# rapidsai/cugraph

Measured on NVIDIA H100. Metric: MTEPS (million traversed edges/sec) PageRank RMAT-24 ef-16, 100 iterations, higher is better.
Workload: dtype f32

## Files before the change

cugraph_b200/csrc/capi_basic.cu:

```cuda
#include "graph.cuh"

#include <cstdlib>
#include <map>
#include <mutex>
#include <unordered_map>
#include <unordered_set>

namespace b200 {
namespace {
std::mutex g_stream_mutex;
std::unordered_map<cudaStream_t, int>& live_streams()
{
  static auto* s = new std::unordered_map<cudaStream_t, int>();
  return *s;
}
struct block_cache_t {
  std::multimap<size_t, void*> blocks;
  size_t total{0};
};
std::unordered_map<cudaStream_t, block_cache_t>& block_caches()
{
  static auto* c = new std::unordered_map<cudaStream_t, block_cache_t>();
  return *c;
}
// ... 37 lines not shown
    cudaDeviceSynchronize();
    e = cudaMallocAsync(&p, bytes, s);
  }
  CUDA_TRY(e);
  *capacity = bytes;
  return p;
}

void block_free(void* p, size_t capacity, cudaStream_t s)
{
  std::lock_guard<std::mutex> lk(g_stream_mutex);
  if (live_streams().count(s) == 0) {
    cudaFree(p);
    return;
  }
  block_cache_t& c = block_caches()[s];
  if (c.total + capacity > kBlockCacheCap) flush_cache_locked(s, c, true);
  if (capacity > kBlockCacheCap) {
    cudaFreeAsync(p, s);
    return;
  }
  c.blocks.emplace(capacity, p);
  c.total += capacity;
}

bool stream_is_live(cudaStream_t s)
{
  std::lock_guard<std::mutex> lk(g_stream_mutex);
  return live_streams().count(s) != 0;
}
void register_stream(cudaStream_t s)
{
  std::lock_guard<std::mutex> lk(g_stream_mutex);
  ++live_streams()[s];
}
void unregister_stream(cudaStream_t s)
{
  std::lock_guard<std::mutex> lk(g_stream_mutex);
  auto live = live_streams().find(s);
  if (live != live_streams().end() && --live->second > 0) return;
  auto it = block_caches().find(s);
  if (it != block_caches().end()) {
    flush_cache_locked(s, it->second, true);
    block_caches().erase(it);
  }
  live_streams().erase(s);
}

namespace {
struct handle_deleter {
  void operator()(handle_impl* h) const
  {
    if (h->pinned) cudaFreeHost(h->pinned);
    if (h->stream && !h->borrowed_stream) cudaStreamDestroy(h->stream);
    delete h;
  }
};

cugraph_resource_handle_t* create_handle(const char* entry, cudaStream_t stream, bool borrowed)
{
  try {
    std::unique_ptr<handle_impl, handle_deleter> h(new handle_impl{});
    h->tune            = tuning_t::from_env();
    h->stream          = stream;
    h->borrowed_stream = borrowed;
    CUDA_TRY(cudaGetDevice(&h->device));
    if (!borrowed) CUDA_TRY(cudaStreamCreateWithFlags(&h->stream, cudaStreamNonBlocking));
    cudaDeviceProp prop{};
    CUDA_TRY(cudaGetDeviceProperties(&prop, h->device));
    h->sm_count = prop.multiProcessorCount;
    h->l2_bytes = static_cast<size_t>(prop.l2CacheSize);
    CUDA_TRY(cudaMallocHost(&h->pinned, 4096));
    cudaMemPool_t pool;
    CUDA_TRY(cudaDeviceGetDefaultMemPool(&pool, h->device));
    uint64_t threshold = UINT64_MAX;
    CUDA_TRY(cudaMemPoolSetAttribute(pool, cudaMemPoolAttrReleaseThreshold, &threshold));
    register_stream(h->stream);
    return reinterpret_cast<cugraph_resource_handle_t*>(h.release());
  } catch (std::exception const& e) {
    std::fprintf(stderr, "%s: %s\n", entry, e.what());
    return nullptr;
  }
}
}
}

using namespace b200;

extern "C" {

const char* cugraph_error_message(const cugraph_error_t* error)
{
  if (error == nullptr) return nullptr;
  return reinterpret_cast<error_impl const*>(error)->message.c_str();
}

void cugraph_error_free(cugraph_error_t* error)
{
  if (error != nullptr) delete reinterpret_cast<error_impl*>(error);
}

cugraph_resource_handle_t* cugraph_create_resource_handle(void* raft_handle)
{
  if (raft_handle != nullptr) {
    std::fprintf(stderr, "cugraph_create_resource_handle: multi-GPU goes through cugraph_b200.mg (torch.distributed) + the "
                         "cugraph_b200_block_* entry points\n");
    return nullptr;
  }
  return create_handle("cugraph_create_resource_handle", nullptr, false);
}

int cugraph_resource_handle_get_comm_size(const cugraph_resource_handle_t*) { return 1; }

int cugraph_resource_handle_get_rank(const cugraph_resource_handle_t*) { return 0; }

void cugraph_free_resource_handle(cugraph_resource_handle_t* handle)
{
  if (!handle) return;
  auto* h = reinterpret_cast<handle_impl*>(handle);
  cudaStreamSynchronize(h->stream);
// ... 248 lines not shown
```

cugraph_b200/csrc/common.cuh:

```cuda
#pragma once

#include <cugraph_c/b200_ext.h>
#include <cugraph_c/graph_functions.h>
#include <cugraph_c/labeling_algorithms.h>
#include <cuda_runtime.h>

#include <algorithm>
#include <cstdint>
#include <cstdio>
#include <cstdlib>
#include <cstring>
#include <stdexcept>
#include <string>
#include <utility>

namespace b200 {

struct error_impl {
  std::string message;
};

struct capi_exception : public std::runtime_error {
  cugraph_error_code_t code;
  capi_exception(cugraph_error_code_t c, std::string const& m) : std::runtime_error(m), code(c) {}
// ... 9 lines not shown
    cudaError_t e__ = (call);                                                                    \
    if (e__ != cudaSuccess) {                                                                    \
      cudaGetLastError();                                                                        \
      throw ::b200::capi_exception(                                                              \
        e__ == cudaErrorMemoryAllocation ? CUGRAPH_ALLOC_ERROR : CUGRAPH_UNKNOWN_ERROR,          \
        std::string("CUDA error ") + cudaGetErrorName(e__) + " at " + __FILE__ + ":" +           \
          std::to_string(__LINE__) + ": " + cudaGetErrorString(e__));                            \
    }                                                                                            \
  } while (0)

template <typename F>
cugraph_error_code_t guarded(cugraph_error_t** error, F&& f)
{
  if (error) *error = nullptr;
  try {
    f();
    return CUGRAPH_SUCCESS;
  } catch (capi_exception const& e) {
    if (error) *error = reinterpret_cast<cugraph_error_t*>(new error_impl{e.what()});
    return e.code;
  } catch (std::bad_alloc const&) {
    if (error) *error = reinterpret_cast<cugraph_error_t*>(new error_impl{"host allocation failed"});
    return CUGRAPH_ALLOC_ERROR;
  } catch (std::exception const& e) {
    if (error) *error = reinterpret_cast<cugraph_error_t*>(new error_impl{e.what()});
    return CUGRAPH_UNKNOWN_ERROR;
  }
}

inline size_t dtype_size(cugraph_data_type_id_t t)
{
  switch (t) {
    case INT8:
    case UINT8:
    case BOOL: return 1;
    case INT16:
    case UINT16: return 2;
    case INT32:
    case UINT32:
    case FLOAT32: return 4;
    case INT64:
    case UINT64:
    case FLOAT64:
    case SIZE_T: return 8;
    default: return 0;
  }
}

struct tuning_t {
  long long sweep_min_edges{1ll << 22};
  bool sweep_bank_order{true};
  int sweep_bands{0};
  int sweep_tail_degree{0};
  double bfs_alpha{40.0}, bfs_beta{24.0};
  bool sssp_adaptive{true};
  double sssp_delta_scale{1.0};
  double sssp_start_div{64.0};
  bool sssp_small_rounds{true};
  int sssp_split_rounds{1};
  unsigned long long sssp_split_min_edges{1ull << 20};
  unsigned long long advance_split_edges{1ull << 31};
  long long offs64_min_edges{1ll << 31};
  bool bfs_trace{false}, sssp_trace{false}, build_trace{false}, scc_trace{false};
  static tuning_t from_env()
  {
    tuning_t t;
    auto get = [](const char* k) { return std::getenv(k); };
    if (auto e = get("CUGRAPH_B200_SWEEP_MIN_EDGES")) t.sweep_min_edges = std::atoll(e);
    if (auto e = get("CUGRAPH_B200_SWEEP_BANK_ORDER")) t.sweep_bank_order = std::atoi(e) != 0;
    if (auto e = get("CUGRAPH_B200_SWEEP_BANDS")) t.sweep_bands = std::max(0, std::atoi(e));
    if (auto e = get("CUGRAPH_B200_SWEEP_TAIL_DEGREE")) t.sweep_tail_degree = std::max(0, std::atoi(e));
    if (auto e = get("CUGRAPH_B200_BFS_ALPHA")) t.bfs_alpha = std::atof(e);
    if (auto e = get("CUGRAPH_B200_BFS_BETA")) t.bfs_beta = std::atof(e);
    if (auto e = get("CUGRAPH_B200_SSSP_ADAPTIVE")) t.sssp_adaptive = std::atoi(e) != 0;
    if (auto e = get("CUGRAPH_B200_SSSP_DELTA_SCALE")) t.sssp_delta_scale = std::atof(e);
    if (auto e = get("CUGRAPH_B200_SSSP_START_DIV")) t.sssp_start_div = std::max(1.0, std::atof(e));
    if (auto e = get("CUGRAPH_B200_SSSP_SMALL_ROUNDS")) t.sssp_small_rounds = std::atoi(e) != 0;
    if (auto e = get("CUGRAPH_B200_SSSP_SPLIT_ROUNDS")) t.sssp_split_rounds = std::max(1, std::atoi(e));
    if (auto e = get("CUGRAPH_B200_SSSP_SPLIT_MIN_EDGES")) t.sssp_split_min_edges = std::strtoull(e, nullptr, 10);
    if (auto e = get("CUGRAPH_B200_ADVANCE_SPLIT_EDGES")) t.advance_split_edges = std::min<unsigned long long>(std::max<unsigned long long>(std::strtoull(e, nullptr, 10), 2ull), 1ull << 31);
    if (auto e = get("CUGRAPH_B200_OFFS64_MIN_EDGES")) t.offs64_min_edges = std::min(std::max(std::atoll(e), 0ll), 1ll << 31);
    t.bfs_trace   = get("CUGRAPH_B200_BFS_TRACE") != nullptr;
    t.sssp_trace  = get("CUGRAPH_B200_SSSP_TRACE") != nullptr;
    t.build_trace = get("CUGRAPH_B200_BUILD_TRACE") != nullptr;
    t.scc_trace   = get("CUGRAPH_B200_SCC_TRACE") != nullptr;
    return t;
  }
};

struct handle_impl {
  tuning_t tune{};
  int device{0};
  cudaStream_t stream{nullptr};
  bool borrowed_stream{false};
  int sm_count{132};
  size_t l2_bytes{0};
  mutable size_t launches{0};
  void* pinned{nullptr};
};

inline handle_impl const& H(const cugraph_resource_handle_t* h)
{
  B200_EXPECTS(h != nullptr, CUGRAPH_INVALID_HANDLE, "resource handle is NULL");
  return *reinterpret_cast<handle_impl const*>(h);
}

inline bool bfs_bottom_up(handle_impl const& h, bool bottom_up, long long n_f, long long prev_n_f, unsigned long long m_f,
                          unsigned long long m_u, long long n_unvisited)
{
  if (!bottom_up && (double)m_f * h.tune.bfs_alpha > (double)m_u && n_f >= prev_n_f) return true;
  if (bottom_up && (double)n_f * h.tune.bfs_beta < (double)n_unvisited && n_f < prev_n_f) return false;
  return bottom_up;
}

bool stream_is_live(cudaStream_t s);
void register_stream(cudaStream_t s);
void unregister_stream(cudaStream_t s);

void* block_alloc(size_t bytes, cudaStream_t s, size_t* capacity);
void block_free(void* p, size_t capacity, cudaStream_t s);

class dbuf {
 public:
  dbuf() = default;
  dbuf(size_t bytes, cudaStream_t s) : bytes_(bytes), stream_(s)
  {
    if (bytes_ > 0) p_ = block_alloc(bytes_, s, &cap_);
  }
  dbuf(dbuf const&)            = delete;
  dbuf& operator=(dbuf const&) = delete;
  dbuf(dbuf&& o) noexcept { swap(o); }
  dbuf& operator=(dbuf&& o) noexcept
  {
    if (this != &o) {
      release();
      swap(o);
    }
    return *this;
  }
  ~dbuf() { release(); }
  void release()
  {
    if (p_) block_free(p_, cap_, stream_);
    p_     = nullptr;
    bytes_ = cap_ = 0;
  }
  void* data() const { return p_; }
// ... 40 lines not shown
};

struct host_array_view_impl {
  void* data{nullptr};
  size_t size{0};
  cugraph_data_type_id_t type{INT32};
  size_t nbytes() const { return size * dtype_size(type); }
};

struct host_array_impl {
  void* data{nullptr};
  size_t size{0};
  cugraph_data_type_id_t type{INT32};
};

inline device_array_view_impl const* V(const cugraph_type_erased_device_array_view_t* v)
{
  return reinterpret_cast<device_array_view_impl const*>(v);
}

inline cugraph_type_erased_device_array_t* wrap_array(dbuf&& b, size_t n, cugraph_data_type_id_t t)
{
  auto* a = new device_array_impl{std::move(b), n, t};
  return reinterpret_cast<cugraph_type_erased_device_array_t*>(a);
}

struct centrality_result_impl {
  device_array_impl* vertices{nullptr};
  device_array_impl* values{nullptr};
  size_t iterations{0};
  bool converged{false};
};

struct paths_result_impl {
  device_array_impl* vertices{nullptr};
  device_array_impl* distances{nullptr};
  device_array_impl* predecessors{nullptr};
};

struct labeling_result_impl {
  device_array_impl* vertices{nullptr};
  device_array_impl* labels{nullptr};
};

constexpr int kBlock = 256;

inline int grid_for(int64_t n, int per_thread = 1, int max_grid = 1 << 20)
{
  const int64_t b = (n + (int64_t)kBlock * per_thread - 1) / ((int64_t)kBlock * per_thread);
  return (int)std::min<int64_t>(std::max<int64_t>(b, 1), std::min(max_grid, 1 << 20));
}

#ifndef B200_HOST_EMU
#define B200_LAUNCH(h, kernel, grid, block, smem, ...)                           \
  do {                                                                           \
    if ((grid) > 0) {                                                            \
      kernel<<<(grid), (block), (smem), (h).stream>>>(__VA_ARGS__);              \
      (h).launches++;                                                            \
    }                                                                            \
  } while (0)
__device__ __forceinline__ bool is_commit_lane() { return (threadIdx.x & 31) == 0; }
#else
#define B200_LAUNCH(h, kernel, grid, block, smem, ...)                           \
  do {                                                                           \
    if ((grid) > 0) {                                                            \
      emu_launch((grid), (block), (size_t)(smem), [&] { kernel(__VA_ARGS__); }); \
      (h).launches++;                                                            \
    }                                                                            \
  } while (0)
inline bool is_commit_lane() { return true; }
#endif

__device__ __forceinline__ double warp_sum(double v)
{
#pragma unroll
  for (int o = 16; o > 0; o >>= 1) v += __shfl_xor_sync(0xffffffffu, v, o);
  return v;
}

inline void check_last(const char* what)
{
  cudaError_t e = cudaGetLastError();
  if (e != cudaSuccess)
    throw capi_exception(CUGRAPH_UNKNOWN_ERROR,
                         std::string("kernel launch failed (") + what + "): " + cudaGetErrorString(e));
}

inline void sync(handle_impl const& h) { CUDA_TRY(cudaStreamSynchronize(h.stream)); }

template <typename T>
T read_back(handle_impl const& h, T const* d)
{
  T v{};
  CUDA_TRY(cudaMemcpyAsync(&v, d, sizeof(T), cudaMemcpyDeviceToHost, h.stream));
  sync(h);
  return v;
}

namespace {

template <typename T>
__global__ void k_fill(T* __restrict__ a, int64_t n, T v)
{
  for (int64_t i = blockIdx.x * (int64_t)blockDim.x + threadIdx.x; i < n; i += (int64_t)gridDim.x * blockDim.x) a[i] = v;
}

template <typename T>
__global__ void k_iota(T* __restrict__ a, int64_t n)
{
  for (int64_t i = blockIdx.x * (int64_t)blockDim.x + threadIdx.x; i < n; i += (int64_t)gridDim.x * blockDim.x) a[i] = (T)i;
}

template <typename T>
__global__ void k_count_negative(T const* __restrict__ a, int64_t n, int* __restrict__ out)
{
  for (int64_t i = blockIdx.x * (int64_t)blockDim.x + threadIdx.x; i < n; i += (int64_t)gridDim.x * blockDim.x)
    if (a[i] < (T)0) atomicAdd(out, 1);
}

__device__ __forceinline__ double block_sum(double v, double* smem)
{
  v = warp_sum(v);
  if ((threadIdx.x & 31) == 0) smem[threadIdx.x >> 5] = v;
  __syncthreads();
// ... 45 lines not shown
```

cugraph_b200/csrc/sweep.cuh:

```cuda
#pragma once
#include "spmv.cuh"
#include "sweep_layout.cuh"

namespace b200 {

constexpr int kSweepThreads = 512;
constexpr int kSweepWarps   = kSweepThreads / 32;
constexpr int kSweepDynSmem = kHotSliceBytes;
constexpr int kTmaPiece     = 16 * 1024;
constexpr int kStealMin     = 12;

#ifndef B200_HOST_EMU
__device__ __forceinline__ uint32_t smem_u32(const void* p) { return (uint32_t)__cvta_generic_to_shared(p); }

__device__ __forceinline__ void mbar_init(uint64_t* bar, unsigned count)
{
  asm volatile("mbarrier.init.shared::cta.b64 [%0], %1;" ::"r"(smem_u32(bar)), "r"(count));
  asm volatile("fence.mbarrier_init.release.cluster;" ::: "memory");
}
__device__ __forceinline__ void mbar_expect_tx(uint64_t* bar, unsigned bytes)
{
  asm volatile("mbarrier.arrive.expect_tx.shared::cta.b64 _, [%0], %1;" ::"r"(smem_u32(bar)), "r"(bytes) : "memory");
}
__device__ __forceinline__ void mbar_wait(uint64_t* bar, unsigned parity)
// ... 559 lines not shown
    else if (r < n_cov) acc[r] = 0.0;
    const T v0 = (T)(q[k].x * alpha + init), v1 = (T)(q[k].y * alpha + init);
    bool paired = false;
    if constexpr (sizeof(T) == 4) {
      if (!row_vertex && r + 1 < n_rows) {
        if (y) *reinterpret_cast<float2*>(y + r) = make_float2(v0, v1);
        if (epi.x_next) epi_row_pair(epi, r, v0, v1, make_float2((float)ow[k][0], (float)ow[k][1]), sums);
        paired = true;
      }
    }
    if (!paired) {
#pragma unroll
      for (int j = 0; j < 2; ++j) {
        if (r + j < n_rows) {
          const int v = row_vertex ? row_vertex[r + j] : r + j;
          store_row(y, epi, v, j ? v1 : v0, epi_in_t<T>{ow[k][j], epi.y_old ? epi.y_old[v] : (T)0}, sums);
        }
      }
    }
  }
  epi_flush(epi, sums);
}

constexpr int kTailThreads = 512;
constexpr int kTailBatch   = 8;

#ifndef B200_HOST_EMU
__device__ __forceinline__ float ld_keep(float const* p, unsigned long long pol)
{
  float v;
  asm("ld.global.nc.L2::cache_hint.f32 %0, [%1], %2;" : "=f"(v) : "l"(p), "l"(pol));
  return v;
}
__device__ __forceinline__ double ld_keep(double const* p, unsigned long long pol)
{
  double v;
  asm("ld.global.nc.L2::cache_hint.f64 %0, [%1], %2;" : "=d"(v) : "l"(p), "l"(pol));
  return v;
}
#else
inline float ld_keep(float const* p, unsigned long long) { return *p; }
inline double ld_keep(double const* p, unsigned long long) { return *p; }
#endif

template <typename T>
struct tail_args_t {
  tail_run_t const* __restrict__ runs;
  int32_t const* __restrict__ ids;
  T const* __restrict__ w;
  T const* __restrict__ x;
  T* __restrict__ y;
  int32_t const* __restrict__ row_vertex;
  int* __restrict__ cursor;
  pr_state_t const* __restrict__ st;
  int n_runs, empty_hi, W;
  double alpha;
  row_epi_t<T> epi;
};

struct tail_unit_t {
  int d, n_tiles, row0, row_end;
  long long base;
};

__device__ __forceinline__ tail_unit_t tail_unit(tail_run_t const* runs, int n_runs, int u)
{
  tail_unit_t t{0, 0, 0, 0, 0};
  if (u >= runs[n_runs].first_unit) return t;
  int r = 0;
  while (u >= runs[r + 1].first_unit) ++r;
  const tail_run_t R = runs[r];
  const int per      = tail_unit_tiles(R.degree);
  const int tile     = (u - R.first_unit) * per;
  t.d                = R.degree;
  const int left     = runs[r + 1].first_tile - R.first_tile - tile;
  t.n_tiles          = left < per ? left : per;
  t.row0             = R.first_row + tile * kTailTile;
  t.row_end          = runs[r + 1].first_row;
  t.base             = R.id_off + (long long)tile * kTailTile * R.degree;
  return t;
}

__device__ __forceinline__ void tail_load(int (&q)[kTailUnitEntries], tail_unit_t const& u, int32_t const* __restrict__ ids,
                                          unsigned long long pol, int lane)
{
  const int n         = u.n_tiles * u.d;
  int32_t const* base = ids + u.base + lane;
#pragma unroll
  for (int j = 0; j < kTailUnitEntries; ++j)
    if (j < n) q[j] = ld_stream_i32(base + j * kTailTile, pol);
}

template <typename T, bool WEIGHTED, int D, bool EPI>
__device__ __forceinline__ void tail_rows(int const (&q)[kTailUnitEntries], tail_unit_t const& u, tail_args_t<T> const& a,
                                          T const* __restrict__ sx, double init, unsigned long long pol, unsigned long long keep,
                                          int lane, epi_sums_t& sums)
{
  constexpr int U = tail_unit_tiles(D);
  T const* wp       = WEIGHTED ? a.w + u.base + lane : nullptr;
#pragma unroll
  for (int t = 0; t < U; ++t) {
    if (t < u.n_tiles) {
      const int row = u.row0 + t * kTailTile + lane;
      const int v   = row < u.row_end ? (a.row_vertex ? a.row_vertex[row] : row) : -1;
      const epi_in_t<T> p = EPI && v >= 0 ? epi_load(a.epi, v) : epi_in_t<T>{(T)0, (T)0};
      double s = 0.0;
#pragma unroll
      for (int k0 = 0; k0 < D; k0 += kTailBatch) {
        double b[kTailBatch];
#pragma unroll
        for (int i = 0; i < kTailBatch; ++i) {
          b[i] = 0.0;
          if (k0 + i < D) {
            const int j = t * D + k0 + i;
            const int c = j < kTailUnitEntries ? q[j] : ld_stream_i32(a.ids + u.base + j * kTailTile + lane, pol);
            T v         = c < a.W ? sx[c] : ld_keep(a.x + c, keep);
            if (WEIGHTED) v *= ld_stream(wp + j * kTailTile);
            b[i] = (double)v;
          }
        }
        s += ((b[0] + b[1]) + (b[2] + b[3])) + ((b[4] + b[5]) + (b[6] + b[7]));
      }
      if (v >= 0) {
        if constexpr (EPI) store_row(a.y, a.epi, v, (T)(s * a.alpha + init), p, sums);
        else a.y[v] = (T)(s * a.alpha + init);
      }
    }
  }
}

template <typename T, bool WEIGHTED, bool EPI, int D = 1>
__device__ __forceinline__ void tail_process(int const (&q)[kTailUnitEntries], tail_unit_t const& u, tail_args_t<T> const& a,
                                             T const* __restrict__ sx, double init, unsigned long long pol,
                                             unsigned long long keep, int lane, epi_sums_t& sums)
{
  if (u.d == D) tail_rows<T, WEIGHTED, D, EPI>(q, u, a, sx, init, pol, keep, lane, sums);
  else if constexpr (D < kTailMaxDegree) tail_process<T, WEIGHTED, EPI, D + 1>(q, u, a, sx, init, pol, keep, lane, sums);
}

template <typename T, bool WEIGHTED, bool EPI>
__global__ void __launch_bounds__(kTailThreads, 1) k_sweep_tail(tail_args_t<T> a)
{
  B200_DYN_SMEM(smem_raw);
  T const* sx = reinterpret_cast<T const*>(smem_raw);
  __shared__ uint64_t bar;
  __shared__ tail_run_t s_run[kTailMaxDegree + 1];
  if (a.st->done) return;
  const unsigned long long pol = make_l2_policy_evict_first(), keep = make_l2_policy_evict_last();
  const int lane = threadIdx.x & 31;
  if (threadIdx.x == 0) {
    mbar_init(&bar, 1);
    load_slice(smem_raw, a.x, 0, a.W, &bar);
  }
  if ((int)threadIdx.x <= a.n_runs) s_run[threadIdx.x] = a.runs[threadIdx.x];
  const double init = a.st->init;
  epi_sums_t sums;
  __syncthreads();
  const int ra = draw_issue(a.cursor, 1, lane, true), rb = draw_issue(a.cursor, 1, lane, true);
  tail_unit_t A = tail_unit(s_run, a.n_runs, draw_get(ra));
  int qa[kTailUnitEntries], qb[kTailUnitEntries];
  tail_load(qa, A, a.ids, pol, lane);
  tail_unit_t B = tail_unit(s_run, a.n_runs, draw_get(rb));
  mbar_wait(&bar, 0);
  while (A.d > 0) {
    tail_load(qb, B, a.ids, pol, lane);
    const int rc = draw_issue(a.cursor, 1, lane, B.d > 0);
    tail_process<T, WEIGHTED, EPI>(qa, A, a, sx, init, pol, keep, lane, sums);
    if (B.d == 0) break;
    const tail_unit_t C = tail_unit(s_run, a.n_runs, draw_get(rc));
    tail_load(qa, C, a.ids, pol, lane);
    const int rd = draw_issue(a.cursor, 1, lane, C.d > 0);
    tail_process<T, WEIGHTED, EPI>(qb, B, a, sx, init, pol, keep, lane, sums);
    A = C;
    B = tail_unit(s_run, a.n_runs, draw_get(rd));
  }
  const int stride = gridDim.x * blockDim.x;
  const int tid    = (int)(blockIdx.x * blockDim.x + threadIdx.x);
  const int lo     = a.runs[a.n_runs].first_row;
  if constexpr (!EPI) {
    for (int r = lo + tid; r < a.empty_hi; r += stride) a.y[a.row_vertex ? a.row_vertex[r] : r] = (T)init;
  } else if (a.row_vertex) {
    for (int r = lo + tid; r < a.empty_hi; r += stride) store_row(a.y, a.epi, a.row_vertex[r], (T)init, sums);
  } else {
    constexpr int kV = 16 / sizeof(T), kEmptyBatch = 4;
    const int v_lo = (lo + kV - 1) / kV, v_hi = a.empty_hi / kV;
    const int s_hi = v_lo < v_hi ? v_lo * kV : a.empty_hi;
    for (int r = lo + tid; r < s_hi; r += stride) store_row(a.y, a.epi, r, (T)init, sums);
    for (int r = (v_lo < v_hi ? v_hi * kV : a.empty_hi) + tid; r < a.empty_hi; r += stride) store_row(a.y, a.epi, r, (T)init, sums);
    const T fill = (T)init;
    for (int i0 = v_lo + tid; i0 < v_hi; i0 += kEmptyBatch * stride) {
      uint4 ow[kEmptyBatch], old[kEmptyBatch];
#pragma unroll
      for (int j = 0; j < kEmptyBatch; ++j) {
        const int i = i0 + j * stride;
        if (i < v_hi) {
          ow[j] = reinterpret_cast<uint4 const*>(a.epi.out_w)[i];
          if (a.epi.y_old) old[j] = reinterpret_cast<uint4 const*>(a.epi.y_old)[i];
        }
      }
#pragma unroll
      for (int j = 0; j < kEmptyBatch; ++j) {
        const int i = i0 + j * stride;
        if (i < v_hi) {
          T w[kV], o[kV], yv[kV], xv[kV];
          std::memcpy(w, &ow[j], 16);
          if (a.epi.y_old) std::memcpy(o, &old[j], 16);
#pragma unroll
          for (int k = 0; k < kV; ++k) {
            yv[k] = fill;
            xv[k] = w[k] == (T)0 ? fill : fill / w[k];
            if (w[k] == (T)0) sums.dangling += (double)fill;
            if (a.epi.y_old) sums.diff += fabs((double)fill - (double)o[k]);
          }
          uint4 qy, qx;
          std::memcpy(&qy, yv, 16);
          std::memcpy(&qx, xv, 16);
          if (a.y) reinterpret_cast<uint4*>(a.y)[i] = qy;
          reinterpret_cast<uint4*>(a.epi.x_next)[i] = qx;
        }
      }
    }
  }
  if constexpr (EPI) epi_flush(a.epi, sums);
}

template <typename T>
void launch_sweep(handle_impl const& h, csx_t const& c, sweep_layout_t const& L, T const* x, T* y, double* acc, double alpha,
                  pr_state_t const* st, bool use_weights, bool covered_rows_only, row_epi_t<T> const& epi)
{
  const bool weighted = use_weights && L.w.data() != nullptr;
  auto* const sweep_kernel = weighted ? k_sweep<T, true> : k_sweep<T, false>;
  auto* const tail_kernel  = epi.x_next ? (weighted ? k_sweep_tail<T, true, true> : k_sweep_tail<T, false, true>)
                                        : (weighted ? k_sweep_tail<T, true, false> : k_sweep_tail<T, false, false>);
  CUDA_TRY(cudaFuncSetAttribute(sweep_kernel, cudaFuncAttributeMaxDynamicSharedMemorySize, kSweepDynSmem));
  sweep_args_t<T> a;
  a.p.ids     = L.ids.as<uint4>();
  a.p.rows    = L.rows.as<int32_t>();
  a.p.w       = L.w.data();
  a.p.acc     = acc;
  a.chunks    = L.chunks.as<sweep_chunk_t>();
  a.phases    = L.phases.as<sweep_phase_t>();
  a.cursor    = L.cursor.as<int>();
  a.x         = x;
  a.st        = st;
  a.W         = L.W;
  a.p.pol     = 0;
  a.p.acc_pol = 0;
  constexpr int kFinishSteps = 8;
  const int32_t finish_rows = covered_rows_only ? L.n_cov : c.n_rows;
  const bool tail           = L.n_str < L.n_cov;
  for (int band = 0; band < L.n_bands; ++band) {
    const int row_hi = band < L.n_bands - 1 ? L.band_row[band + 1] : (tail ? L.n_str : finish_rows);
    const int row_lo = L.band_row[band];
    a.cta_phase      = L.cta_phase.as<int32_t>() + (size_t)band * L.n_cta;
    a.ph_lo          = L.band_phase[band];
    a.ph_hi          = L.band_phase[band + 1];
    B200_LAUNCH(h, sweep_kernel, L.n_cta, kSweepThreads, kSweepDynSmem, a);
    const int n_ph = a.ph_hi - a.ph_lo + (band == L.n_bands - 1 && tail ? 1 : 0);
    const int n    = std::max((row_hi - row_lo + 2 * kFinishSteps - 1) / (2 * kFinishSteps), n_ph);
    B200_LAUNCH(h, (k_sweep_finish<T, kFinishSteps>), (std::max(n, 1) + 255) / 256, 256, 0, acc, row_lo, L.n_str, row_hi, y,
                c.row_vertex.as<int32_t>(), alpha, L.cursor.as<int>() + a.ph_lo, n_ph, st, epi);
  }
  if (tail) {
    tail_args_t<T> t;
    t.runs       = L.tail_run.as<tail_run_t>();
    t.ids        = L.tail_ids.as<int32_t>();
    t.w          = weighted ? L.tail_w.as<T>() : nullptr;
    t.x          = x;
    t.y          = y;
    t.row_vertex = c.row_vertex.as<int32_t>();
    t.cursor     = L.cursor.as<int>() + L.n_phases;
    t.st         = st;
    t.n_runs     = L.n_tail_runs;
    t.empty_hi   = finish_rows;
    t.W          = L.W;
    t.alpha      = alpha;
    t.epi        = epi;
    const int units  = L.tail_runs.back().first_unit;
    const int blocks = std::max(1, std::min(h.sm_count, (units + kTailThreads / 32 - 1) / (kTailThreads / 32)));
    CUDA_TRY(cudaFuncSetAttribute(tail_kernel, cudaFuncAttributeMaxDynamicSharedMemorySize, kSweepDynSmem));
    B200_LAUNCH(h, tail_kernel, blocks, kTailThreads, kSweepDynSmem, t);
  }
}

}
```

cugraph_b200/csrc/sweep_layout.cu:

```cuda
#include "sweep_layout.cuh"
#include "staging.cuh"

#include <thrust/iterator/counting_iterator.h>

namespace b200 {

namespace {


__global__ void k_hot_row_starts(int32_t const* __restrict__ off, int32_t n_cov, uint8_t* __restrict__ flag)
{
  for (int64_t r = blockIdx.x * (int64_t)blockDim.x + threadIdx.x; r < n_cov; r += (int64_t)gridDim.x * blockDim.x) flag[(size_t)off[r]] = 1;
}

__global__ void k_hot_heads(int32_t const* __restrict__ idx, long long nnz, int W, uint8_t* __restrict__ flag)
{
  for (long long e = blockIdx.x * (long long)blockDim.x + threadIdx.x; e < nnz; e += (long long)gridDim.x * blockDim.x) {
    if (e > 0 && !flag[e] && idx[e] / W != idx[e - 1] / W) flag[e] = 1;
  }
}

constexpr int kHotPieceSlots   = 8;
constexpr int kHotPieceEntries = kHotPieceSlots * kHotSlot;

// ... 310 lines not shown
    }
  }
}

void build_tail_layout(handle_impl const& h, csx_t const& c, int32_t nv, size_t es, sweep_layout_t& L)
{
  dbuf d_below = make_dbuf<int32_t>(kTailMaxDegree + 2, h.stream);
  B200_LAUNCH(h, k_tail_run_bounds, 1, 64, 0, c.offsets.as<int32_t>(), L.n_str, L.n_cov, d_below.as<int32_t>());
  int32_t below[kTailMaxDegree + 2];
  CUDA_TRY(cudaMemcpyAsync(below, d_below.data(), sizeof(below), cudaMemcpyDeviceToHost, h.stream));
  sync(h);
  tail_run_t at{0, L.n_str, 0, 0, 0};
  for (int d = kTailMaxDegree; d >= 1; --d) {
    const int32_t lo = below[d + 1], hi = below[d];
    if (hi <= lo) continue;
    B200_EXPECTS(lo == at.first_row, CUGRAPH_UNKNOWN_ERROR, "tail rows are not degree-descending");
    at.degree = d;
    L.tail_runs.push_back(at);
    const int32_t tiles = (hi - lo + kTailTile - 1) / kTailTile;
    at.first_row = hi;
    at.first_tile += tiles;
    at.first_unit += (tiles + tail_unit_tiles(d) - 1) / tail_unit_tiles(d);
    at.id_off += (int64_t)tiles * kTailTile * d;
  }
  B200_EXPECTS(at.first_row == L.n_cov, CUGRAPH_UNKNOWN_ERROR, "tail rows of in-degree >= the bound or 0");
  at.degree     = 0;
  L.n_tail_runs = (int)L.tail_runs.size();
  L.tail_runs.push_back(at);
  L.tail_run = make_dbuf<tail_run_t>(L.tail_runs.size(), h.stream);
  CUDA_TRY(cudaMemcpyAsync(L.tail_run.data(), L.tail_runs.data(), sizeof(tail_run_t) * L.tail_runs.size(), cudaMemcpyHostToDevice,
                           h.stream));
  L.tail_ids = make_dbuf<int32_t>((size_t)std::max<int64_t>(at.id_off, 1), h.stream);
  const bool weighted = c.weights.data() != nullptr;
  if (weighted) L.tail_w = dbuf((size_t)std::max<int64_t>(at.id_off, 1) * es, h.stream);
  const int64_t threads = (int64_t)at.first_tile * kTailTile;
  if (es == 4)
    B200_LAUNCH(h, (k_tail_fill<float>), grid_for(threads), kBlock, 0, L.tail_run.as<tail_run_t>(), L.n_tail_runs,
                c.offsets.as<int32_t>(), c.indices.as<int32_t>(), c.weights.as<float>(), nv, L.tail_ids.as<int32_t>(), L.tail_w.as<float>());
  else
    B200_LAUNCH(h, (k_tail_fill<double>), grid_for(threads), kBlock, 0, L.tail_run.as<tail_run_t>(), L.n_tail_runs,
                c.offsets.as<int32_t>(), c.indices.as<int32_t>(), c.weights.as<double>(), nv, L.tail_ids.as<int32_t>(), L.tail_w.as<double>());
  check_last("sweep tail layout");
  sync(h);
}

constexpr double kBandL2Share = 0.5;

int sweep_bands(handle_impl const& h, int32_t n_str)
{
  const int most = std::max(1, (int)(((int64_t)n_str + kBandRowAlign - 1) / kBandRowAlign));
  int P          = h.tune.sweep_bands;
  if (P <= 0) P = h.l2_bytes ? (int)std::ceil(8.0 * n_str / (kBandL2Share * (double)h.l2_bytes)) : 1;
  return std::min(std::max(P, 1), most);
}

int sweep_stream_bin(handle_impl const& h, csx_t const& c)
{
  int bound = h.tune.sweep_tail_degree;
  if (bound <= 0) bound = c.nnz >= kSweepTailMinEdges ? kSweepTailDegree : 1;
  int k = 0;
  while (kSegThreshold[k] > bound) ++k;
  return k;
}

std::unique_ptr<sweep_layout_t> build_sweep_layout(handle_impl const& h, csx_t const& c, int32_t nv, size_t es)
{
  phase_trace tr(h);
  const int W         = (int)(kHotSliceBytes / es) - kHotZeroPad;
  const int32_t n_cov = c.seg[kNumSeg - 2];
  const int32_t n_str = c.seg[sweep_stream_bin(h, c)];
  if (n_str <= 0) return nullptr;
  const int B         = (int)(((int64_t)nv + W - 1) / W);
  const int64_t nnz   = read_back(h, c.offsets.as<int32_t>() + n_str);
  auto L              = std::make_unique<sweep_layout_t>();
  L->W = W; L->B = B; L->n_cov = n_cov; L->n_str = n_str; L->nnz = c.nnz;
  int32_t const* idx = c.indices.as<int32_t>();
  const int asked         = sweep_bands(h, n_str);
  const int32_t band_rows = (int32_t)((((int64_t)n_str + asked - 1) / asked + kBandRowAlign - 1) / kBandRowAlign * kBandRowAlign);
  const int n_bands       = (int)(((int64_t)n_str + band_rows - 1) / band_rows);
  L->n_bands              = n_bands;
  for (int b = 0; b <= n_bands; ++b) L->band_row.push_back((int32_t)std::min<int64_t>((int64_t)b * band_rows, n_str));

  dbuf flag = make_dbuf<uint8_t>(nnz, h.stream);
  CUDA_TRY(cudaMemsetAsync(flag.data(), 0, nnz, h.stream));
  B200_LAUNCH(h, k_hot_row_starts, grid_for(n_str), kBlock, 0, c.offsets.as<int32_t>(), n_str, flag.as<uint8_t>());
  B200_LAUNCH(h, k_hot_heads, grid_for(nnz, 4, h.sm_count * 32), kBlock, 0, idx, (long long)nnz, W, flag.as<uint8_t>());
  dbuf head_pos = make_dbuf<int32_t>(nnz, h.stream);
  const int64_t n_segs64 = select_flagged<int32_t, thrust::counting_iterator<int32_t>>(
    h, thrust::counting_iterator<int32_t>(0), flag.as<uint8_t>(), head_pos.as<int32_t>(), nnz);
  flag.release();
  const int32_t n_segs = (int32_t)n_segs64;
  tr.mark("sweep layout: segment heads");

  dbuf seg_row = make_dbuf<int32_t>(n_segs, h.stream), seg_pieces = make_dbuf<int32_t>((size_t)n_segs + 1, h.stream);
  dbuf piece_off = make_dbuf<int32_t>((size_t)n_segs + 1, h.stream);
  B200_LAUNCH(h, k_hot_segment_info, grid_for((int64_t)n_segs + 1), kBlock, 0, head_pos.as<int32_t>(), n_segs,
              (long long)nnz, c.offsets.as<int32_t>(), n_str, seg_row.as<int32_t>(), seg_pieces.as<int32_t>());
  exclusive_scan_i32(h, seg_pieces.as<int32_t>(), piece_off.as<int32_t>(), (int64_t)n_segs + 1);
  const int32_t n_pieces = read_back(h, piece_off.as<int32_t>() + n_segs);
  seg_pieces.release();
  L->n_pieces = n_pieces;
  dbuf piece_key = make_dbuf<uint32_t>(n_pieces, h.stream), piece_key2 = make_dbuf<uint32_t>(n_pieces, h.stream);
  dbuf piece_start = make_dbuf<int32_t>(n_pieces, h.stream), piece_len = make_dbuf<int32_t>(n_pieces, h.stream);
  dbuf piece_row = make_dbuf<int32_t>(n_pieces, h.stream);
  B200_LAUNCH(h, k_hot_emit_pieces, grid_for(n_segs), kBlock, 0, head_pos.as<int32_t>(), n_segs, (long long)nnz, idx, W, B,
              band_rows, seg_row.as<int32_t>(), piece_off.as<int32_t>(), piece_key.as<uint32_t>(), piece_start.as<int32_t>(),
              piece_len.as<int32_t>(), piece_row.as<int32_t>());
  head_pos.release();
  seg_row.release();
  piece_off.release();
  tr.mark("sweep layout: pieces");

  const int n_keys = n_bands * B * kNumKinds;
  dbuf perm = make_dbuf<uint32_t>(n_pieces, h.stream), perm2 = make_dbuf<uint32_t>(n_pieces, h.stream);
  B200_LAUNCH(h, k_iota<uint32_t>, grid_for(n_pieces, 4), kBlock, 0, perm.as<uint32_t>(), (int64_t)n_pieces);
  sort_pairs<uint32_t, uint32_t>(h, piece_key.as<uint32_t>(), piece_key2.as<uint32_t>(), perm.as<uint32_t>(),
                                 perm2.as<uint32_t>(), n_pieces, 0, bits_for(n_keys + 1));
  dbuf class_start = make_dbuf<int32_t>((size_t)n_keys + 1, h.stream);
  B200_LAUNCH(h, k_hot_class_starts, grid_for(n_keys + 1), kBlock, 0, piece_key2.as<uint32_t>(), n_pieces, n_keys,
              class_start.as<int32_t>());
  std::vector<int32_t> cstart((size_t)n_keys + 1);
  CUDA_TRY(cudaMemcpyAsync(cstart.data(), class_start.data(), sizeof(int32_t) * cstart.size(), cudaMemcpyDeviceToHost, h.stream));
  sync(h);
  piece_key.release();
  piece_key2.release();
  perm.release();
  tr.mark("sweep layout: kind sort");
  if (tr.on) {
    int edges[] = {0, 1, 4, 16, 64, 160, B};
    std::fprintf(stderr, "[sweep] B=%d W=%d rows=%d (tail %d rows, %lld edges) nnz=%lld segments=%d pieces=%d bands=%d of %d rows\n",
                 B, W, n_str, n_cov - n_str, (long long)(c.nnz - nnz), (long long)nnz, n_segs, n_pieces, n_bands, band_rows);
    for (int k = 0; k + 1 < 7; ++k) {
      const int b0 = std::min(edges[k], B), b1 = std::min(edges[k + 1], B);
      if (b1 <= b0) continue;
      std::fprintf(stderr, "[sweep] blocks [%d,%d) pieces by kind S Q H F1..F8:", b0, b1);
      for (int kind = 0; kind < kNumKinds; ++kind) {
        long long np = 0;
        for (int band = 0; band < n_bands; ++band)
          for (int b = b0; b < b1; ++b) np += cstart[(band * B + b) * kNumKinds + kind + 1] - cstart[(band * B + b) * kNumKinds + kind];
        std::fprintf(stderr, " %lld", np);
      }
      std::fprintf(stderr, "\n");
    }
  }

  sweep_plan_t plan;
  if (!plan_sweep(cstart, n_bands, B, h.sm_count, plan)) return nullptr;
  L->band_phase = plan.band_phase;
  L->n_steprows = plan.n_steprows;
  L->n_rowslots = plan.n_rowslots;
  L->n_chunks   = (int32_t)plan.chunks.size();
  L->n_phases   = (int32_t)plan.phases.size();
  L->n_cta      = plan.n_cta;
  L->chunks     = make_dbuf<sweep_chunk_t>(std::max<size_t>(plan.chunks.size(), 1), h.stream);
  L->phases     = make_dbuf<sweep_phase_t>(std::max<size_t>(plan.phases.size(), 1), h.stream);
  L->cta_phase  = make_dbuf<int32_t>(plan.cta_phase.size(), h.stream);
  dbuf d_fills  = make_dbuf<sweep_fill_t>(std::max<size_t>(plan.fills.size(), 1), h.stream);
  if (!plan.chunks.empty()) {
    CUDA_TRY(cudaMemcpyAsync(L->chunks.data(), plan.chunks.data(), sizeof(sweep_chunk_t) * plan.chunks.size(), cudaMemcpyHostToDevice, h.stream));
    CUDA_TRY(cudaMemcpyAsync(L->phases.data(), plan.phases.data(), sizeof(sweep_phase_t) * plan.phases.size(), cudaMemcpyHostToDevice, h.stream));
    CUDA_TRY(cudaMemcpyAsync(d_fills.data(), plan.fills.data(), sizeof(sweep_fill_t) * plan.fills.size(), cudaMemcpyHostToDevice, h.stream));
  }
  CUDA_TRY(cudaMemcpyAsync(L->cta_phase.data(), plan.cta_phase.data(), sizeof(int32_t) * plan.cta_phase.size(), cudaMemcpyHostToDevice, h.stream));
  sync(h);
  L->cursor = make_dbuf<int>(L->n_phases + 1, h.stream);
  CUDA_TRY(cudaMemsetAsync(L->cursor.data(), 0, sizeof(int) * (L->n_phases + 1), h.stream));

  L->ids  = make_dbuf<uint4>((size_t)std::max<int64_t>(L->n_steprows, 1) * 32, h.stream);
  L->rows = make_dbuf<int32_t>(std::max<int64_t>(L->n_rowslots, 1), h.stream);
  const bool weighted = c.weights.data() != nullptr;
  if (weighted) L->w = dbuf((size_t)std::max<int64_t>(L->n_steprows, 1) * 32 * kHotSlot * es, h.stream);
  L->bank_order = h.tune.sweep_bank_order && es == 4;
  if (!plan.chunks.empty()) {
    const int grid = (int)plan.chunks.size();
    if (es == 4 && L->bank_order)
      B200_LAUNCH(h, (k_sweep_fill<float, true>), grid, kFillWarps * 32, 0, L->chunks.as<sweep_chunk_t>(), d_fills.as<sweep_fill_t>(),
                  perm2.as<int32_t>(), piece_start.as<int32_t>(), piece_len.as<int32_t>(), piece_row.as<int32_t>(), idx,
                  c.weights.as<float>(), W, L->ids.as<uint4>(), L->w.as<float>(), L->rows.as<int32_t>());
    else if (es == 4)
      B200_LAUNCH(h, (k_sweep_fill<float, false>), grid, kFillWarps * 32, 0, L->chunks.as<sweep_chunk_t>(), d_fills.as<sweep_fill_t>(),
                  perm2.as<int32_t>(), piece_start.as<int32_t>(), piece_len.as<int32_t>(), piece_row.as<int32_t>(), idx,
                  c.weights.as<float>(), W, L->ids.as<uint4>(), L->w.as<float>(), L->rows.as<int32_t>());
    else
      B200_LAUNCH(h, (k_sweep_fill<double, false>), grid, kFillWarps * 32, 0, L->chunks.as<sweep_chunk_t>(), d_fills.as<sweep_fill_t>(),
                  perm2.as<int32_t>(), piece_start.as<int32_t>(), piece_len.as<int32_t>(), piece_row.as<int32_t>(), idx,
                  c.weights.as<double>(), W, L->ids.as<uint4>(), L->w.as<double>(), L->rows.as<int32_t>());
  }
  check_last("sweep layout");
  sync(h);
  tr.mark("sweep layout: fill");
  if (n_str < n_cov) {
    build_tail_layout(h, c, nv, es, *L);
    tr.mark("sweep layout: tail");
    if (tr.on) {
      std::fprintf(stderr, "[sweep] tail: %d runs, %d tiles, %d units, %.1f MB of ids\n", L->n_tail_runs,
                   L->tail_runs.back().first_tile, L->tail_runs.back().first_unit, (double)L->tail_runs.back().id_off * 4 / 1e6);
    }
  }
  if (tr.on) {
    std::fprintf(stderr, "[sweep] %lld step-rows = %.1f MB of ids, %lld row slots = %.1f MB, %d chunks, %d phases, %d CTAs\n",
                 (long long)L->n_steprows, (double)L->n_steprows * 512 / 1e6, (long long)L->n_rowslots,
                 (double)L->n_rowslots * 4 / 1e6, L->n_chunks, L->n_phases, L->n_cta);
    for (int band = 0; band < n_bands; ++band) {
      const int p0 = plan.band_phase[band], p1 = plan.band_phase[band + 1];
      const int c0 = p1 > p0 ? plan.phases[p0].chunk_begin : 0, c1 = p1 > p0 ? plan.phases[p1 - 1].chunk_end : 0;
      std::fprintf(stderr, "[sweep] band %d rows [%d,%d): %d pieces, %d chunks, %d phases = slice loads\n", band,
                   L->band_row[band], L->band_row[band + 1], cstart[(band + 1) * B * kNumKinds] - cstart[band * B * kNumKinds],
                   c1 - c0, p1 - p0);
    }
  }
  return L;
}

}

bool debug_plan_sweep(std::vector<int32_t> const& cstart, int n_bands, int B, int sm_count, int64_t totals[3],
                      std::vector<int32_t>& chunks4, std::vector<int32_t>& fills4, std::vector<int32_t>& phases4,
                      std::vector<int32_t>& cta_phase, std::vector<int32_t>& band_phase)
{
  sweep_plan_t P;
  if (!plan_sweep(cstart, n_bands, B, sm_count, P)) return false;
  totals[0] = P.n_steprows; totals[1] = P.n_rowslots; totals[2] = P.n_cta;
  for (auto const& x : P.chunks) chunks4.insert(chunks4.end(), {x.sr_begin, x.row_begin, x.n_groups, x.kind});
  for (auto const& x : P.fills) fills4.insert(fills4.end(), {x.piece_begin, x.piece_end, x.block, x.pad});
  for (auto const& x : P.phases) phases4.insert(phases4.end(), {x.block, x.chunk_begin, x.chunk_end, x.pad});
  cta_phase  = P.cta_phase;
  band_phase = P.band_phase;
  return true;
}

sweep_layout_t const* sweep_layout(handle_impl const& h, csx_t const& c, int32_t n_vertices, size_t elem_size)
{
  if (!c.sweep) c.sweep = std::make_unique<sweep_cache_t>();
  auto& slot = c.sweep->of(elem_size);
  if (slot.tried) return slot.layout.get();
  slot.tried = true;
  if (!c.degree_sorted || c.seg[kNumSeg - 2] <= 0 || c.nnz < h.tune.sweep_min_edges || c.offs64 || c.nnz >= (1ll << 31) - 4096)
    return nullptr;
  slot.layout = build_sweep_layout(h, c, n_vertices, elem_size);
  return slot.layout.get();
}

csx_t::csx_t()  = default;
csx_t::~csx_t() = default;

}

extern "C" cugraph_error_code_t cugraph_b200_debug_plan_sweep_bands(const int32_t* class_start, int n_bands, int n_blocks,
                                                                    int sm_count, int64_t* totals, int32_t* chunks,
                                                                    int32_t* fills, size_t chunks_capacity, size_t* n_chunks,
                                                                    int32_t* phases, size_t phases_capacity, size_t* n_phases,
                                                                    int32_t* cta_phase, size_t cta_capacity,
                                                                    int32_t* band_phase, cugraph_error_t** error)
{
  using namespace b200;
// ... 33 lines not shown
```

cugraph_b200/csrc/sweep_layout.cuh:

```cuda
#pragma once
#include "graph.cuh"

namespace b200 {

constexpr int kHotSliceBytes = 192 * 1024;
constexpr int kHotZeroPad    = 64;
constexpr int kHotSlot       = 8;

constexpr int kBandRowAlign = 512;

constexpr int kSweepTailDegree         = 16;
constexpr long long kSweepTailMinEdges = 1ll << 24;

constexpr int kNumKinds = 11;
constexpr int kKindS = 0, kKindQ = 1, kKindH = 2, kKindF1 = 3;
__host__ __device__ __forceinline__ int kind_steps(int kind) { return kind < kKindF1 ? 1 : kind - 2; }
__host__ __device__ __forceinline__ int kind_pieces(int kind) { return kind == kKindS ? 256 : (kind == kKindQ ? 128 : (kind == kKindH ? 64 : 32)); }
__host__ __device__ __forceinline__ int kind_chunk_groups(int kind)
{
  return kind == kKindS ? 2 : (kind == kKindQ ? 4 : (kind == kKindH ? 4 : (kind == kKindF1 ? 6 : (kind == kKindF1 + 1 ? 3 : (kind <= kKindF1 + 3 ? 2 : 1)))));
}

struct sweep_chunk_t {
  int32_t sr_begin;
  int32_t row_begin;
  int32_t n_groups;
  int32_t kind;
};
struct sweep_phase_t {
  int32_t block;
  int32_t chunk_begin;
  int32_t chunk_end;
  int32_t pad;
};

constexpr int kTailTile        = 32;
constexpr int kTailUnitEntries = 24;
constexpr int kTailMaxDegree   = 31;
__host__ __device__ constexpr int tail_unit_tiles(int d) { return d >= kTailUnitEntries ? 1 : kTailUnitEntries / d; }

struct tail_run_t {
  int32_t degree;
  int32_t first_row;
  int32_t first_tile;
  int32_t first_unit;
  int64_t id_off;
};

struct sweep_layout_t {
  int W{0};
  int B{0};
  int32_t n_cov{0};
  int32_t n_str{0};
  int64_t nnz{0};
  bool bank_order{false};
  int64_t n_steprows{0};
  int64_t n_rowslots{0};
  int64_t n_pieces{0};
  dbuf ids;
  dbuf w;
  dbuf rows;
  dbuf chunks;
  dbuf phases;
  dbuf cta_phase;
  dbuf cursor;
  int32_t n_chunks{0};
  int32_t n_phases{0};
  int n_cta{0};
  int n_bands{1};
  std::vector<int32_t> band_row;
  std::vector<int32_t> band_phase;
  int n_tail_runs{0};
  std::vector<tail_run_t> tail_runs;
  dbuf tail_run;
  dbuf tail_ids;
  dbuf tail_w;
};

struct sweep_cache_t {
  struct slot_t { bool tried{false}; std::unique_ptr<sweep_layout_t> layout; } slot[2];
  slot_t& of(size_t elem_size) { return slot[elem_size == 4 ? 0 : 1]; }
};

sweep_layout_t const* sweep_layout(handle_impl const& h, csx_t const& c, int32_t n_vertices, size_t elem_size);

}
```

Before: 403,900.

## Run low-degree tail kernel concurrently on a side stream with SM split

Launches the sparse-tail SpMV kernel on a separate stream forked from the main stream, so it runs alongside the streamed sweep kernels. A cost model divides the SMs between the two parts, and the sweep plan is built for the SMs left over. Double-buffered cursors, each reset by the opposite launch, let successive tail launches avoid a separate reset. This adds event fork/join overhead per iteration and depends on the cost-model estimate; a poor split could leave SMs idle.

```diff
diff --git a/cugraph_b200/csrc/capi_basic.cu b/cugraph_b200/csrc/capi_basic.cu
--- a/cugraph_b200/csrc/capi_basic.cu
+++ b/cugraph_b200/csrc/capi_basic.cu
@@ -113,6 +113,9 @@
   void operator()(handle_impl* h) const
   {
     if (h->pinned) cudaFreeHost(h->pinned);
+    if (h->fork) cudaEventDestroy(h->fork);
+    if (h->join) cudaEventDestroy(h->join);
+    if (h->side) cudaStreamDestroy(h->side);
     if (h->stream && !h->borrowed_stream) cudaStreamDestroy(h->stream);
     delete h;
   }
@@ -127,6 +130,9 @@
     h->borrowed_stream = borrowed;
     CUDA_TRY(cudaGetDevice(&h->device));
     if (!borrowed) CUDA_TRY(cudaStreamCreateWithFlags(&h->stream, cudaStreamNonBlocking));
+    CUDA_TRY(cudaStreamCreateWithFlags(&h->side, cudaStreamNonBlocking));
+    CUDA_TRY(cudaEventCreateWithFlags(&h->fork, cudaEventDisableTiming));
+    CUDA_TRY(cudaEventCreateWithFlags(&h->join, cudaEventDisableTiming));
     cudaDeviceProp prop{};
     CUDA_TRY(cudaGetDeviceProperties(&prop, h->device));
     h->sm_count = prop.multiProcessorCount;
diff --git a/cugraph_b200/csrc/common.cuh b/cugraph_b200/csrc/common.cuh
--- a/cugraph_b200/csrc/common.cuh
+++ b/cugraph_b200/csrc/common.cuh
@@ -85,6 +85,7 @@
   bool sweep_bank_order{true};
   int sweep_bands{0};
   int sweep_tail_degree{0};
+  int sweep_tail_sms{-1};
   double bfs_alpha{40.0}, bfs_beta{24.0};
   bool sssp_adaptive{true};
   double sssp_delta_scale{1.0};
@@ -103,6 +104,7 @@
     if (auto e = get("CUGRAPH_B200_SWEEP_BANK_ORDER")) t.sweep_bank_order = std::atoi(e) != 0;
     if (auto e = get("CUGRAPH_B200_SWEEP_BANDS")) t.sweep_bands = std::max(0, std::atoi(e));
     if (auto e = get("CUGRAPH_B200_SWEEP_TAIL_DEGREE")) t.sweep_tail_degree = std::max(0, std::atoi(e));
+    if (auto e = get("CUGRAPH_B200_SWEEP_TAIL_SMS")) t.sweep_tail_sms = std::atoi(e);
     if (auto e = get("CUGRAPH_B200_BFS_ALPHA")) t.bfs_alpha = std::atof(e);
     if (auto e = get("CUGRAPH_B200_BFS_BETA")) t.bfs_beta = std::atof(e);
     if (auto e = get("CUGRAPH_B200_SSSP_ADAPTIVE")) t.sssp_adaptive = std::atoi(e) != 0;
@@ -126,6 +128,8 @@
   int device{0};
   cudaStream_t stream{nullptr};
   bool borrowed_stream{false};
+  cudaStream_t side{nullptr};
+  cudaEvent_t fork{nullptr}, join{nullptr};
   int sm_count{132};
   size_t l2_bytes{0};
   mutable size_t launches{0};
@@ -272,24 +276,26 @@
 }
 
 #ifndef B200_HOST_EMU
-#define B200_LAUNCH(h, kernel, grid, block, smem, ...)                           \
+#define B200_LAUNCH_ON(h, s, kernel, grid, block, smem, ...)                     \
   do {                                                                           \
     if ((grid) > 0) {                                                            \
-      kernel<<<(grid), (block), (smem), (h).stream>>>(__VA_ARGS__);              \
+      kernel<<<(grid), (block), (smem), (s)>>>(__VA_ARGS__);                     \
       (h).launches++;                                                            \
     }                                                                            \
   } while (0)
 __device__ __forceinline__ bool is_commit_lane() { return (threadIdx.x & 31) == 0; }
 #else
-#define B200_LAUNCH(h, kernel, grid, block, smem, ...)                           \
+#define B200_LAUNCH_ON(h, s, kernel, grid, block, smem, ...)                     \
   do {                                                                           \
     if ((grid) > 0) {                                                            \
+      (void)(s);                                                                 \
       emu_launch((grid), (block), (size_t)(smem), [&] { kernel(__VA_ARGS__); }); \
       (h).launches++;                                                            \
     }                                                                            \
   } while (0)
 inline bool is_commit_lane() { return true; }
 #endif
+#define B200_LAUNCH(h, kernel, grid, block, smem, ...) B200_LAUNCH_ON(h, (h).stream, kernel, grid, block, smem, __VA_ARGS__)
 
 __device__ __forceinline__ double warp_sum(double v)
 {
diff --git a/cugraph_b200/csrc/sweep.cuh b/cugraph_b200/csrc/sweep.cuh
--- a/cugraph_b200/csrc/sweep.cuh
+++ b/cugraph_b200/csrc/sweep.cuh
@@ -635,6 +635,7 @@
   T* __restrict__ y;
   int32_t const* __restrict__ row_vertex;
   int* __restrict__ cursor;
+  int* __restrict__ spent;
   pr_state_t const* __restrict__ st;
   int n_runs, empty_hi, W;
   double alpha;
@@ -728,6 +729,7 @@
   T const* sx = reinterpret_cast<T const*>(smem_raw);
   __shared__ uint64_t bar;
   __shared__ tail_run_t s_run[kTailMaxDegree + 1];
+  if (blockIdx.x == 0 && threadIdx.x == 0) *a.spent = 0;
   if (a.st->done) return;
   const unsigned long long pol = make_l2_policy_evict_first(), keep = make_l2_policy_evict_last();
   const int lane = threadIdx.x & 31;
@@ -816,6 +818,36 @@
   auto* const tail_kernel  = epi.x_next ? (weighted ? k_sweep_tail<T, true, true> : k_sweep_tail<T, false, true>)
                                         : (weighted ? k_sweep_tail<T, true, false> : k_sweep_tail<T, false, false>);
   CUDA_TRY(cudaFuncSetAttribute(sweep_kernel, cudaFuncAttributeMaxDynamicSharedMemorySize, kSweepDynSmem));
+  const int32_t finish_rows = covered_rows_only ? L.n_cov : c.n_rows;
+  const bool tail           = L.n_str < L.n_cov;
+  const bool split          = tail && L.tail_sms > 0;
+  auto launch_tail = [&](cudaStream_t s, int sms) {
+    tail_args_t<T> t;
+    const unsigned slot = L.tail_sweeps++ & 1u;
+    t.runs       = L.tail_run.as<tail_run_t>();
+    t.ids        = L.tail_ids.as<int32_t>();
+    t.w          = weighted ? L.tail_w.as<T>() : nullptr;
+    t.x          = x;
+    t.y          = y;
+    t.row_vertex = c.row_vertex.as<int32_t>();
+    t.cursor     = L.cursor.as<int>() + L.n_phases + slot;
+    t.spent      = L.cursor.as<int>() + L.n_phases + (slot ^ 1u);
+    t.st         = st;
+    t.n_runs     = L.n_tail_runs;
+    t.empty_hi   = finish_rows;
+    t.W          = L.W;
+    t.alpha      = alpha;
+    t.epi        = epi;
+    const int units  = L.tail_runs.back().first_unit;
+    const int blocks = std::max(1, std::min(sms, (units + kTailThreads / 32 - 1) / (kTailThreads / 32)));
+    CUDA_TRY(cudaFuncSetAttribute(tail_kernel, cudaFuncAttributeMaxDynamicSharedMemorySize, kSweepDynSmem));
+    B200_LAUNCH_ON(h, s, tail_kernel, blocks, kTailThreads, kSweepDynSmem, t);
+  };
+  if (split) {
+    CUDA_TRY(cudaEventRecord(h.fork, h.stream));
+    CUDA_TRY(cudaStreamWaitEvent(h.side, h.fork, 0));
+    launch_tail(h.side, L.tail_sms);
+  }
   sweep_args_t<T> a;
   a.p.ids     = L.ids.as<uint4>();
   a.p.rows    = L.rows.as<int32_t>();
@@ -830,8 +862,6 @@
   a.p.pol     = 0;
   a.p.acc_pol = 0;
   constexpr int kFinishSteps = 8;
-  const int32_t finish_rows = covered_rows_only ? L.n_cov : c.n_rows;
-  const bool tail           = L.n_str < L.n_cov;
   for (int band = 0; band < L.n_bands; ++band) {
     const int row_hi = band < L.n_bands - 1 ? L.band_row[band + 1] : (tail ? L.n_str : finish_rows);
     const int row_lo = L.band_row[band];
@@ -839,31 +869,17 @@
     a.ph_lo          = L.band_phase[band];
     a.ph_hi          = L.band_phase[band + 1];
     B200_LAUNCH(h, sweep_kernel, L.n_cta, kSweepThreads, kSweepDynSmem, a);
-    const int n_ph = a.ph_hi - a.ph_lo + (band == L.n_bands - 1 && tail ? 1 : 0);
+    const int n_ph = a.ph_hi - a.ph_lo;
     const int n    = std::max((row_hi - row_lo + 2 * kFinishSteps - 1) / (2 * kFinishSteps), n_ph);
     B200_LAUNCH(h, (k_sweep_finish<T, kFinishSteps>), (std::max(n, 1) + 255) / 256, 256, 0, acc, row_lo, L.n_str, row_hi, y,
                 c.row_vertex.as<int32_t>(), alpha, L.cursor.as<int>() + a.ph_lo, n_ph, st, epi);
   }
-  if (tail) {
-    tail_args_t<T> t;
-    t.runs       = L.tail_run.as<tail_run_t>();
-    t.ids        = L.tail_ids.as<int32_t>();
-    t.w          = weighted ? L.tail_w.as<T>() : nullptr;
-    t.x          = x;
-    t.y          = y;
-    t.row_vertex = c.row_vertex.as<int32_t>();
-    t.cursor     = L.cursor.as<int>() + L.n_phases;
-    t.st         = st;
-    t.n_runs     = L.n_tail_runs;
-    t.empty_hi   = finish_rows;
-    t.W          = L.W;
-    t.alpha      = alpha;
-    t.epi        = epi;
-    const int units  = L.tail_runs.back().first_unit;
-    const int blocks = std::max(1, std::min(h.sm_count, (units + kTailThreads / 32 - 1) / (kTailThreads / 32)));
-    CUDA_TRY(cudaFuncSetAttribute(tail_kernel, cudaFuncAttributeMaxDynamicSharedMemorySize, kSweepDynSmem));
-    B200_LAUNCH(h, tail_kernel, blocks, kTailThreads, kSweepDynSmem, t);
-  }
-}
-
-}
+  if (split) {
+    CUDA_TRY(cudaEventRecord(h.join, h.side));
+    CUDA_TRY(cudaStreamWaitEvent(h.stream, h.join, 0));
+  } else if (tail) {
+    launch_tail(h.stream, h.sm_count);
+  }
+}
+
+}
diff --git a/cugraph_b200/csrc/sweep_layout.cu b/cugraph_b200/csrc/sweep_layout.cu
--- a/cugraph_b200/csrc/sweep_layout.cu
+++ b/cugraph_b200/csrc/sweep_layout.cu
@@ -386,6 +386,26 @@
   int P          = h.tune.sweep_bands;
   if (P <= 0) P = h.l2_bytes ? (int)std::ceil(8.0 * n_str / (kBandL2Share * (double)h.l2_bytes)) : 1;
   return std::min(std::max(P, 1), most);
+}
+
+constexpr double kTailEntryCost = 1.4;
+constexpr double kTailRowEntries = 1.0, kTailEmptyEntries = 0.25;
+
+int sweep_tail_sms(handle_impl const& h, std::vector<int32_t> const& cstart, int n_bands, int B, int64_t tail_entries,
+                   int64_t tail_rows, int64_t empty_rows, double* stream_cost, double* tail_cost)
+{
+  double stream = 0.0;
+  for (int key = 0; key < n_bands * B * kNumKinds; ++key) {
+    const int kind = key % kNumKinds, ppg = kind_pieces(kind);
+    stream += (double)(((int64_t)cstart[key + 1] - cstart[key] + ppg - 1) / ppg) * sweep_group_cost(kind);
+  }
+  const double tail = kTailEntryCost * ((double)tail_entries + kTailRowEntries * (double)tail_rows + kTailEmptyEntries * (double)empty_rows);
+  *stream_cost = stream;
+  *tail_cost   = tail;
+  if (tail_rows <= 0 || h.sm_count < 2) return 0;
+  int k = h.tune.sweep_tail_sms;
+  if (k < 0) k = (int)std::lround(h.sm_count * tail / std::max(stream + tail, 1.0));
+  return std::min(std::max(k, 0), h.sm_count - 1);
 }
 
 int sweep_stream_bin(handle_impl const& h, csx_t const& c)
@@ -478,8 +498,10 @@
     }
   }
 
+  double stream_cost = 0.0, tail_cost = 0.0;
+  L->tail_sms = sweep_tail_sms(h, cstart, n_bands, B, c.nnz - nnz, n_cov - n_str, c.n_rows - n_cov, &stream_cost, &tail_cost);
   sweep_plan_t plan;
-  if (!plan_sweep(cstart, n_bands, B, h.sm_count, plan)) return nullptr;
+  if (!plan_sweep(cstart, n_bands, B, h.sm_count - L->tail_sms, plan)) return nullptr;
   L->band_phase = plan.band_phase;
   L->n_steprows = plan.n_steprows;
   L->n_rowslots = plan.n_rowslots;
@@ -497,8 +519,8 @@
   }
   CUDA_TRY(cudaMemcpyAsync(L->cta_phase.data(), plan.cta_phase.data(), sizeof(int32_t) * plan.cta_phase.size(), cudaMemcpyHostToDevice, h.stream));
   sync(h);
-  L->cursor = make_dbuf<int>(L->n_phases + 1, h.stream);
-  CUDA_TRY(cudaMemsetAsync(L->cursor.data(), 0, sizeof(int) * (L->n_phases + 1), h.stream));
+  L->cursor = make_dbuf<int>(L->n_phases + 2, h.stream);
+  CUDA_TRY(cudaMemsetAsync(L->cursor.data(), 0, sizeof(int) * (L->n_phases + 2), h.stream));
 
   L->ids  = make_dbuf<uint4>((size_t)std::max<int64_t>(L->n_steprows, 1) * 32, h.stream);
   L->rows = make_dbuf<int32_t>(std::max<int64_t>(L->n_rowslots, 1), h.stream);
@@ -535,6 +557,9 @@
     std::fprintf(stderr, "[sweep] %lld step-rows = %.1f MB of ids, %lld row slots = %.1f MB, %d chunks, %d phases, %d CTAs\n",
                  (long long)L->n_steprows, (double)L->n_steprows * 512 / 1e6, (long long)L->n_rowslots,
                  (double)L->n_rowslots * 4 / 1e6, L->n_chunks, L->n_phases, L->n_cta);
+    std::fprintf(stderr, "[sweep] split: tail on %d of %d SMs%s (cost: stream %.4g, tail %.4g = %.1f %%)\n", L->tail_sms,
+                 h.sm_count, h.tune.sweep_tail_sms >= 0 ? ", forced" : "", stream_cost, tail_cost,
+                 100.0 * tail_cost / std::max(stream_cost + tail_cost, 1.0));
     for (int band = 0; band < n_bands; ++band) {
       const int p0 = plan.band_phase[band], p1 = plan.band_phase[band + 1];
       const int c0 = p1 > p0 ? plan.phases[p0].chunk_begin : 0, c1 = p1 > p0 ? plan.phases[p1 - 1].chunk_end : 0;
diff --git a/cugraph_b200/csrc/sweep_layout.cuh b/cugraph_b200/csrc/sweep_layout.cuh
--- a/cugraph_b200/csrc/sweep_layout.cuh
+++ b/cugraph_b200/csrc/sweep_layout.cuh
@@ -67,6 +67,8 @@
   int32_t n_chunks{0};
   int32_t n_phases{0};
   int n_cta{0};
+  int tail_sms{0};
+  mutable unsigned tail_sweeps{0};
   int n_bands{1};
   std::vector<int32_t> band_row;
   std::vector<int32_t> band_phase;
```

After: 439,600 (median of 6 runs). 1.09x the previous value.
